# jstrom2002/Mini-OpenCL-Raytracer

Measured on AMD Instinct MI355X. Metric: Mrays/s (3840x2160 Cornell box, 8 spp, 9 bounces), higher is better.
Workload: dtype f32

## Files before the change

include/rt_hip.h:

```cpp
#ifndef RT_HIP_H
#define RT_HIP_H

#include <stddef.h>
#include <stdint.h>

#include "rt_cl_types.h"
#include "rt_status.h"

#ifdef __cplusplus
extern "C" {
#endif

typedef struct rt_context_s* rt_context;
typedef struct rt_mem_s* rt_mem;
typedef struct rt_kernel_s* rt_kernel;

#define RT_MEM_READ_WRITE (1u << 0)
#define RT_MEM_WRITE_ONLY (1u << 1)
#define RT_MEM_READ_ONLY (1u << 2)
#define RT_MEM_COPY_HOST_PTR (1u << 5)

enum rt_kernel_arg {
    RT_ARG_BUFFER_OUT = 0,
    RT_ARG_BUFFER_SCENE = 1,
// ... 329 lines not shown
typedef struct rt_rect {
    uint64_t img_offset, img_pitch, width, rows, stage_offset;
} rt_rect;
int rtBandPackPlan(unsigned width, unsigned height, unsigned period, unsigned phase, rt_rect* rects,
                   int capacity, int* n_rects, size_t* staging_bytes);

#define RT_PINNED_OP_RCP 0
#define RT_PINNED_OP_DIV 1
#define RT_PINNED_OP_SQRT 2
#define RT_PINNED_OP_RSQRT 3
#define RT_PINNED_OP_POW 4
#define RT_PINNED_OP_SIN 5
#define RT_PINNED_OP_COS 6
int rtDiagPinnedMath(int device_index, int op, const float* a, const float* b, float* out, size_t n);

const char* rtGetBuildInfo(void);

#ifdef __cplusplus
}
#endif

#endif
```

mini-opencl-raytracer_amd/clrt/_native.py:

```python
from __future__ import annotations

import ctypes
import os

import numpy as np

_PKG_ROOT = os.path.dirname(os.path.dirname(os.path.abspath(__file__)))
LIB_DIR = os.path.join(_PKG_ROOT, "lib")
HIP_LIB_PATH = os.environ.get("RT_HIP_LIB") or os.path.join(LIB_DIR, "librt_hip.so")
SCENE_LIB_PATH = os.path.join(LIB_DIR, "librt_scene.so")

RT_SUCCESS = 0
_ERROR_NAMES = {
    0: "CL_SUCCESS", -1: "CL_DEVICE_NOT_FOUND", -4: "CL_MEM_OBJECT_ALLOCATION_FAILURE",
    -5: "CL_OUT_OF_RESOURCES", -6: "CL_OUT_OF_HOST_MEMORY", -30: "CL_INVALID_VALUE",
    -33: "CL_INVALID_DEVICE", -34: "CL_INVALID_CONTEXT", -36: "CL_INVALID_COMMAND_QUEUE",
    -37: "CL_INVALID_HOST_PTR", -38: "CL_INVALID_MEM_OBJECT", -46: "CL_INVALID_KERNEL_NAME",
    -48: "CL_INVALID_KERNEL", -49: "CL_INVALID_ARG_INDEX", -50: "CL_INVALID_ARG_VALUE",
    -51: "CL_INVALID_ARG_SIZE", -52: "CL_INVALID_KERNEL_ARGS", -59: "CL_INVALID_OPERATION",
    -61: "CL_INVALID_BUFFER_SIZE", -63: "CL_INVALID_GLOBAL_WORK_SIZE",
    -1001: "RT_FILE_NOT_FOUND", -1002: "RT_PARSE_ERROR",
}


# ... 250 lines not shown
    "rtCommGetRank": (ctypes.c_int, [_vp, ctypes.POINTER(ctypes.c_int), ctypes.POINTER(ctypes.c_int)]),
    "rtCommShardKernel": (ctypes.c_int, [_vp, _vp]),
    "rtCommSetTransport": (ctypes.c_int, [_vp, ctypes.c_int]),
    "rtCommGetTransport": (ctypes.c_int, [_vp, ctypes.POINTER(ctypes.c_int), ctypes.POINTER(ctypes.c_int)]),
    "rtCommGetStatus": (ctypes.c_int, [_vp, ctypes.POINTER(CommStatus)]),
    "rtCommSetOption": (ctypes.c_int, [_vp, ctypes.c_int, ctypes.c_int]),
    "rtCommEnqueueGatherBands": (ctypes.c_int, [ctypes.POINTER(_vp), ctypes.POINTER(_vp), ctypes.c_int, ctypes.c_uint,
                                                ctypes.c_uint, ctypes.c_int, _vp]),
    "rtCommAllReduceF64": (ctypes.c_int, [ctypes.POINTER(_vp), ctypes.c_int, ctypes.POINTER(ctypes.c_double),
                                          ctypes.c_int, ctypes.c_int]),
    "rtCommBarrier": (ctypes.c_int, [ctypes.POINTER(_vp), ctypes.c_int]),
    "rtBandPackPlan": (ctypes.c_int, [ctypes.c_uint, ctypes.c_uint, ctypes.c_uint, ctypes.c_uint, ctypes.POINTER(Rect),
                                      ctypes.c_int, ctypes.POINTER(ctypes.c_int), ctypes.POINTER(ctypes.c_size_t)]),
    "rtGetBuildInfo": (ctypes.c_char_p, []),
    "rtDiagPinnedMath": (ctypes.c_int, [ctypes.c_int, ctypes.c_int, _vp, _vp, _vp, ctypes.c_size_t]),
}
HIP_EXPORTS = tuple(_HIP_PROTOS)

_SCENE_PROTOS = {
    "rtsLoadOBJ": (ctypes.c_int, [ctypes.c_char_p, ctypes.c_uint, ctypes.POINTER(_vp)]),
    "rtsLoadOBJUnbuilt": (ctypes.c_int, [ctypes.c_char_p, ctypes.POINTER(_vp)]),
    "rtsBuildFromTriangles": (ctypes.c_int, [_vp, ctypes.c_size_t, _vp, ctypes.c_size_t, ctypes.c_uint,
                                             ctypes.POINTER(_vp)]),
    "rtsGetTriangles": (ctypes.c_int, [_vp, ctypes.POINTER(_vp), ctypes.POINTER(ctypes.c_size_t)]),
    "rtsGetNodes": (ctypes.c_int, [_vp, ctypes.POINTER(_vp), ctypes.POINTER(ctypes.c_size_t)]),
    "rtsGetMaterials": (ctypes.c_int, [_vp, ctypes.POINTER(_vp), ctypes.POINTER(ctypes.c_size_t)]),
    "rtsGetTreeStats": (ctypes.c_int, [_vp, ctypes.POINTER(ctypes.c_uint), ctypes.POINTER(ctypes.c_uint),
                                       ctypes.POINTER(ctypes.c_uint)]),
    "rtsFromArrays": (ctypes.c_int, [_vp, ctypes.c_size_t, _vp, ctypes.c_size_t, _vp, ctypes.c_size_t,
                                     ctypes.c_uint, ctypes.POINTER(_vp)]),
# ... 36 lines not shown
    return _load(SCENE_LIB_PATH, _SCENE_PROTOS)


PINNED_OPS = {"rcp": 0, "div": 1, "sqrt": 2, "rsqrt": 3, "pow": 4, "sin": 5, "cos": 6}


def pinned_math(op: str, a, b=None, device: int = 0) -> np.ndarray:
    a = np.ascontiguousarray(a, dtype=np.float32)
    bb = None if b is None else np.ascontiguousarray(np.broadcast_to(np.float32(b) if np.isscalar(b) else b, a.shape),
                                                     dtype=np.float32)
    out = np.empty_like(a)
    check(hip_lib().rtDiagPinnedMath(int(device), PINNED_OPS[op], a.ctypes.data,
                                     None if bb is None else bb.ctypes.data, out.ctypes.data, a.size),
          f"pinned math {op}")
    return out
```

mini-opencl-raytracer_amd/csrc/rt_capi.cpp:

```cpp
#include <hip/hip_runtime.h>

#include <algorithm>
#include <limits>
#include <cstdlib>
#include <cstring>
#include <mutex>
#include <new>
#include <vector>

#include "../../include/rt_cl_types.h"
#include "../../include/rt_hip.h"
#include "rt_adaptive.hpp"
#include "rt_adaptive_plan.hpp"
#include "rt_bvh.hpp"
#include "rt_denoise.hpp"
#include "rt_denoise_plan.hpp"
#include "rt_denoise_samples.hpp"
#include "rt_device_scene.hpp"
#include "rt_internal.hpp"
#include "rt_kernel_state.hpp"
#include "rt_kernels.hpp"
#include "rt_launch_plan.hpp"
#include "rt_motion_launch.hpp"
#include "rt_motion_plan.hpp"
// ... 1739 lines not shown
    int count = 0;
    if (hipGetDeviceCount(&count) != hipSuccess || count == 0) return RT_DEVICE_NOT_FOUND;
    if (device_index < 0 || device_index >= count) return RT_INVALID_DEVICE;
    hipError_t e = hipSetDevice(device_index);
    float* d = nullptr;
    const size_t bytes = n * sizeof(float);
    if (e == hipSuccess) e = hipMalloc(reinterpret_cast<void**>(&d), 3 * bytes);
    if (e == hipSuccess) e = hipMemcpy(d, a, bytes, hipMemcpyHostToDevice);
    if (e == hipSuccess && two) e = hipMemcpy(d + n, b, bytes, hipMemcpyHostToDevice);
    if (e == hipSuccess) e = rtk::launch_pinned_math(op, d, d + n, d + 2 * n, n, nullptr);
    if (e == hipSuccess) e = hipMemcpy(out, d + 2 * n, bytes, hipMemcpyDeviceToHost);
    if (d) (void)hipFree(d);
    return map_hip(e);
}

const char* rtGetBuildInfo(void) {
    return "librt_hip: KernelEntry for gfx950 (HIP), math modes pinned|devicelib|shipped, scene in LDS or HBM";
}

}
```

mini-opencl-raytracer_amd/csrc/rt_kernels.hip:

```cpp
#include "rt_kernel_pick.hpp"

#pragma clang fp contract(off)

namespace rtk {

template <bool kStats, bool kBofs, int kMode>
__global__ __launch_bounds__(256) __attribute__((amdgpu_waves_per_eu(RT_STEP_DEVICELIB_WAVES, 8)))
void kernel_entry_step_devicelib_lds(KernelArgs a) {
    step_body<MathDeviceLib, true, kStats, kBofs, false, kMode>(a);
}
template <bool kStats, int kMode>
__global__ __launch_bounds__(256) __attribute__((amdgpu_waves_per_eu(RT_STEP_GLOBAL_WAVES, 8)))
void kernel_entry_step_devicelib_global(KernelArgs a) {
    step_body<MathDeviceLib, false, kStats, false, false, kMode>(a);
}
template <bool kStats, int kMode>
__global__ __launch_bounds__(256) __attribute__((amdgpu_waves_per_eu(RT_STEP_GOCT_WAVES, 8)))
void kernel_entry_step_devicelib_goct(KernelArgs a) {
    step_body<MathDeviceLib, true, kStats, false, true, kMode>(a);
}
#ifndef RT_STEP_PINNED_WAVES
#define RT_STEP_PINNED_WAVES 5
#endif
template <bool kLdsScene, bool kStats, bool kBofs, bool kGlobalOct, int kMode>
// ... 53 lines not shown
            case Walk::LdsB: return kernel_entry_step_pinned<true, S, true, false, kMode>;
            case Walk::GlobalOct: return kernel_entry_step_pinned<true, S, false, true, kMode>;
            default: return kernel_entry_step_pinned<false, S, false, false, kMode>;
        }
    }
};

template <class M>
__global__ __launch_bounds__(256) RT_ACCUM_OCC void accum_frames(KernelArgs a, const uint32_t* key) {
    accum_frames_body<M>(a, key);
}
template <class M>
__global__ void accum_key(KernelArgs a, uint32_t* key) {
    accum_key_body<M>(a, key);
}

static const Policy& policy(int math) {
    static const Policy devicelib = {pick_entry<MathDeviceLib>,   wf_pick<MathDeviceLib>,  query_pick<MathDeviceLib>,
                                     accum_frames<MathDeviceLib>, accum_key<MathDeviceLib>, camera_rays<MathDeviceLib>,
                                     pack_mats,
                                     hit_surfaces<MathDeviceLib, false>, hit_surfaces<MathDeviceLib, true>,
                                     trace_pick<MathDeviceLib>, camera_paths<MathDeviceLib>,
                                     camera_paths_for<MathDeviceLib>, sample_pick<MathDeviceLib>,
                                     motion_pick<MathDeviceLib>};
    static const Policy pinned = {pick_entry<MathPinned>,   wf_pick<MathPinned>,  query_pick<MathPinned>,
                                  accum_frames<MathPinned>, accum_key<MathPinned>, camera_rays<MathPinned>,
                                  pack_mats,
                                  hit_surfaces<MathPinned, false>, hit_surfaces<MathPinned, true>,
                                     trace_pick<MathPinned>, camera_paths<MathPinned>,
                                     camera_paths_for<MathPinned>, sample_pick<MathPinned>,
                                     motion_pick<MathPinned>};
    return math == MathShipped::kId ? shipped_policy() : math == MathDeviceLib::kId ? devicelib : pinned;
}

hipError_t launch_kernel_entry(const KernelArgs& a, const Variant& v, unsigned grid, size_t smem, hipStream_t st) {
    hipLaunchKernelGGL(policy(v.math).entry(v), dim3(grid), dim3(256), smem, st, a);
    return hipGetLastError();
}

hipError_t launch_accum_frames(const KernelArgs& a, int math, uint32_t* key, hipStream_t st) {
    const Policy& p = policy(math);
    const dim3 grid((a.nTiles + kAccumWgWaves - 1u) / kAccumWgWaves);
    hipLaunchKernelGGL(p.accum_key, dim3(1), dim3(64), 0, st, a, key);
    hipLaunchKernelGGL(p.accum_frames, grid, dim3(64 * kAccumWgWaves), 0, st, a, key);
    return hipGetLastError();
}
// ... 91 lines not shown
    if (i >= n) return;
    const float x = a[i];
    float r;
    switch (op) {
        case 0: r = MathPinned::rcp(x); break;
        case 1: r = MathPinned::div(x, b[i]); break;
        case 2: r = MathPinned::sqrt(x); break;
        case 3: r = MathPinned::rsqrt(x); break;
        case 4: r = MathPinned::pow(x, b[i]); break;
        case 5: r = MathPinned::sin(x); break;
        default: r = MathPinned::cos(x); break;
    }
    out[i] = r;
}

hipError_t launch_pinned_math(int op, const float* a, const float* b, float* out, size_t n, hipStream_t st) {
    if (n) hipLaunchKernelGGL(pinned_math_kernel, dim3((unsigned)((n + 255) / 256)), dim3(256), 0, st, op, a, b, out, n);
    return hipGetLastError();
}

hipError_t launch_pack(const rt_cl_triangle* tris, uint32_t n_tris, float4* pt, float4* ps,
                       const rt_cl_material* mats, uint32_t n_mats, float4* pm, hipStream_t st) {
    if (n_tris) hipLaunchKernelGGL(pack_tris, dim3((n_tris + 255) / 256), dim3(256), 0, st, tris, pt, n_tris);
    if (n_tris) hipLaunchKernelGGL(pack_shade, dim3((n_tris + 255) / 256), dim3(256), 0, st, tris, ps, n_tris);
    if (n_mats) hipLaunchKernelGGL(pack_mats, dim3((n_mats + 255) / 256), dim3(256), 0, st, mats, pm, n_mats);
    if (n_mats)
        hipLaunchKernelGGL(shipped_policy().pack_mats, dim3((n_mats + 255) / 256), dim3(256), 0, st, mats,
                           pm + 4 * (size_t)n_mats, n_mats);
    return hipGetLastError();
}
// ... 4 lines not shown
```

mini-opencl-raytracer_amd/csrc/rt_kernels.hpp:

```cpp
#pragma once

#include <hip/hip_runtime.h>
#include <stdint.h>

#include "../../include/rt_cl_types.h"
#include "rt_layout.hpp"
#include "rt_temporal_math.hpp"

namespace rtk {

struct KernelArgs {
    float4* result;
    const rt_cl_triangle* trisFull;
    const rt_cl_material* materials;
    const float4* packedTris;
    const float4* octNodes;
    const float4* gNodes;
    const float4* shadeTris;
    const float4* shadeMats;
    uint32_t nNodes, nTris, nMats;
    uint32_t octStride;
    uint32_t octB;
    uint32_t octRecords;
    uint32_t nTop;
// ... 110 lines not shown
struct SurfaceArgs {
    const float4* rays;
    const float4* hits;
    float4* out;
    uint32_t first, count;
    uint32_t accFirst;
    uint32_t accLast;
    float inv;
};
using SurfaceKernelFn = void (*)(KernelArgs, SurfaceArgs);
hipError_t launch_surfaces(const KernelArgs& a, const SurfaceArgs& s, int math, bool accumulate, unsigned grid,
                           hipStream_t st);

hipError_t launch_kernel_entry(const KernelArgs& a, const Variant& v, unsigned grid, size_t smem, hipStream_t st);
hipError_t launch_accum_frames(const KernelArgs& a, int math, uint32_t* key, hipStream_t st);
hipError_t launch_pinned_math(int op, const float* a, const float* b, float* out, size_t n, hipStream_t st);
hipError_t launch_pack(const rt_cl_triangle* tris, uint32_t n_tris, float4* pt, float4* ps,
                       const rt_cl_material* mats, uint32_t n_mats, float4* pm, hipStream_t st);

enum class Family : int { Entry, WfExtend, WfShade, Query, Trace, Sample, Motion };
struct OccupancyCache {
    struct Entry {
        int blocks;
        size_t smem;
    };
    Entry e[(int)Family::Motion + 1][kVariantSlots] = {};
    int get(Family f, const Variant& v, size_t smem);
};

struct Policy {
    KernelFn (*entry)(const Variant&);
    WfKernels (*wavefront)(const Variant&);
    QueryKernelFn (*query)(const Variant&);
    void (*accum_frames)(KernelArgs, const uint32_t*);
    void (*accum_key)(KernelArgs, uint32_t*);
    void (*camera_rays)(KernelArgs, float4*, uint32_t);
    void (*pack_mats)(const rt_cl_material*, float4*, uint32_t);
    SurfaceKernelFn surfaces, surfaces_accum;
    TraceKernelFn (*trace)(const Variant&);
    void (*camera_paths)(KernelArgs, float4*, uint32_t*, uint32_t);
    void (*camera_paths_for)(KernelArgs, const uint32_t*, uint32_t, uint32_t, float4*, uint32_t*);
    SampleKernelFn (*sample)(const Variant&);
    MotionKernelFn (*motion)(const Variant&);
};
const Policy& shipped_policy();
#ifndef RT_SPECIALIZE_FUSED
#define RT_SPECIALIZE_FUSED 1
#endif

}
```

mini-opencl-raytracer_amd/csrc/rt_kernels_body.hpp:

```cpp
#pragma once

#include <hip/hip_runtime.h>
#include <stdint.h>

#include "../../include/rt_cl_types.h"
#include "rt_kernels.hpp"
#include "rt_math.hpp"

#pragma clang fp contract(off)

#ifndef RT_STEP_DEVICELIB_WAVES
#define RT_STEP_DEVICELIB_WAVES 5
#endif
#ifndef RT_STEP_GLOBAL_WAVES
#define RT_STEP_GLOBAL_WAVES 6
#endif
#ifndef RT_STEP_GOCT_WAVES
#define RT_STEP_GOCT_WAVES 5
#endif

namespace rtk {

constexpr float kTwoPi = 6.28318530718f;
constexpr float kInvPi = 0.31830988618f;
// ... 518 lines not shown
    }
    return F3{M::max(radiance.x, 0.0f), M::max(radiance.y, 0.0f), M::max(radiance.z, 0.0f)};
}

template <class M>
__device__ __forceinline__ F3 gamma_out(uint32_t frameCount, F3 old, F3 rad) {
    if (frameCount == 0)
        return F3{M::pow(rad.x, 0.45454545f), M::pow(rad.y, 0.45454545f), M::pow(rad.z, 0.45454545f)};
    const float fm1 = (float)(frameCount - 1), fc = (float)frameCount;
    const F3 lin{M::pow(old.x, 2.2f), M::pow(old.y, 2.2f), M::pow(old.z, 2.2f)};
    const F3 num = madd<M>(lin, fm1, rad);
    const F3 acc{M::div(num.x, fc), M::div(num.y, fc), M::div(num.z, fc)};
    return F3{M::pow(acc.x, 0.454545f), M::pow(acc.y, 0.454545f), M::pow(acc.z, 0.454545f)};
}

template <class M>
__device__ __forceinline__ void finish_color(const KernelArgs& a, uint32_t gid, F3 rad) {
    F3 old = f3s(0.0f);
    if (a.frameCount != 0) {
        const float4 o = a.result[gid];
        old = F3{o.x, o.y, o.z};
    }
    const F3 out = gamma_out<M>(a.frameCount, old, rad);
    a.result[gid] = make_float4(out.x, out.y, out.z, 0.0f);
}

template <class M>
__device__ __forceinline__ void finish_pixel(const KernelArgs& a, uint32_t gid, F3 rad, int32_t pid,
                                             float pt) {
    finish_color<M>(a, gid, rad);
    if (a.hitIds) {
        a.hitIds[gid] = pid;
        a.hitT[gid] = pt;
    }
}

__device__ __forceinline__ unsigned long long wave_sum(uint32_t v) {
    unsigned long long x = v;
// ... 133 lines not shown

constexpr uint32_t kIdle = 0, kTrav = 1, kLeaf = 2, kShade = 3, kDone = 4;
constexpr uint32_t kNotWalking = 0x80000000u;

__device__ __forceinline__ uint32_t lane_rank(unsigned long long m) {
    return __builtin_amdgcn_mbcnt_hi((uint32_t)(m >> 32), __builtin_amdgcn_mbcnt_lo((uint32_t)m, 0u));
}

constexpr uint32_t kFinishSlots = 64;
static_assert(kFinishWaveBytes == kFinishSlots * 16, "finish queue layout");

template <class M>
__device__ __forceinline__ void finish_queued(const KernelArgs& a, const float4* fq, uint32_t n, uint32_t lane) {
    if (lane < n) {
        const float4 e = fq[lane];
        finish_color<M>(a, __float_as_uint(e.w), F3{e.x, e.y, e.z});
    }
}
#ifndef RT_PRIO_SHADE
#define RT_PRIO_SHADE 1
#endif
#ifndef RT_NODE_BURST
#define RT_NODE_BURST 7
#endif
#ifndef RT_TIMELINE
#define RT_TIMELINE 0
#endif
#ifndef RT_TIMELINE_DIV
#define RT_TIMELINE_DIV 1
#endif
#ifndef RT_TRI_BURST
#define RT_TRI_BURST 4
#endif
#ifndef RT_WTRI_BURST
#define RT_WTRI_BURST 2
#endif


// ... 131 lines not shown
    auto rootW = [&](uint32_t sgn) -> uint32_t { return kWalk ? __umul24(sgn, octStride16) : 0u; };
    if (kGlobalOct) __syncthreads();

    const F3 camPos{a.camPos[0], a.camPos[1], a.camPos[2]};
    const F3 camFront{a.camFront[0], a.camFront[1], a.camFront[2]};
    const F3 camUp{a.camUp[0], a.camUp[1], a.camUp[2]};
    const float angle = M::tan(0.5f * (45.0f * 3.1415f / 180.0f));
    const uint32_t bounces = (uint32_t)a.lightBounces;
    const uint32_t nVis = fused && kViewCull ? a.visTiles : a.nTiles;
    const uint32_t total = nVis * 64u * (fused ? a.nFrames : 1u);
    const float krad = M::max(madd<M>(1.0f, 0.5f * a.skyboxIntensity, 0.0f), 0.0f);
    float k_old = 0.0f, k_out = 0.0f;
    if (!fused && a.pfKeyIn) {
        k_old = __uint_as_float(*a.pfKeyIn);
        k_out = __uint_as_float(__builtin_amdgcn_readfirstlane(
            __float_as_uint(gamma_out<M>(a.frameCount, f3s(k_old), f3s(krad)).x)));
        if (blockIdx.x == 0 && tid == 0) *a.pfKeyOut = __float_as_uint(k_out);
    }
    const uint32_t rowEnd = a.rowBegin + a.rowCount;
    const int lane = tid & 63;
    const uint32_t kRefillMin = a.refillMin;
    const uint32_t kShadeMin = a.shadeMin;

    extern __shared__ __attribute__((aligned(16))) float4 smem[];
    float4* fq = smem + lds_scene_f4<kLdsScene, kGlobalOct>(a) + (uint32_t)(tid >> 6) * kFinishSlots;
    uint32_t fq_n = 0;
    constexpr bool kRing = kLdsScene && !kGlobalOct;
    float4* ring_d = smem + lds_scene_f4<kLdsScene, kGlobalOct>(a) + (fused ? 0u : 4u * kFinishSlots) +
                     (uint32_t)(tid >> 6) * (fused ? kRingWaveBytes / 16u : kRingWaveBytesPf / 16u);
    float4* ring_i = ring_d + kRingSlots;
    uint32_t* ring_g = reinterpret_cast<uint32_t*>(ring_d + (fused ? 2u : 1u) * kRingSlots);
// ... 291 lines not shown
            if (n_trav + n_leaf == 0u) break;
            if (n_end >= kShadeMin) break;
            const bool leaf_step = n_leaf * a.stepWeightNode > n_trav * a.stepWeightLeaf;
            if (kStats) {
                u_shadew += n_end;
                u_freew += popc_ballot(state == kIdle || state == kDone);
                u_other += leaf_step ? n_trav : n_leaf;
                if (leaf_step) {
                    ++u_tsteps;
                    u_tlanes += n_leaf;
                } else {
                    ++u_nsteps;
                    u_nlanes += n_trav;
                }
            }
            constexpr int kNodeBurst = kGlobalOct ? RT_ONODE_BURST : kLdsScene ? RT_NODE_BURST : RT_GNODE_BURST;
            constexpr int kTriBurst = kGlobalOct ? RT_OTRI_BURST : kLdsScene ? RT_TRI_BURST : RT_GTRI_BURST;
            if (!leaf_step) {
#pragma unroll
                for (int rep = 0; rep < kNodeBurst; ++rep) {
                    if (kLdsScene) {
#if RT_LDS_CONFLICTS
                        if (kStats && !kGlobalOct) {
                            const bool act = cur < kLeafMin;
                            const uint32_t i = kWalk ? cur >> 4 : __umul24(ray.sgn, a.octStride) + cur;
                            lds_model(act, i, i & 15u, true, lm[0], lm[1]);
                            const uint32_t strides[2] = {43u, 48u};
                            for (int v = 0; v < 2; ++v) {
                                const uint32_t iv = ray.sgn * strides[v] + (kWalk ? (cur >> 4) - ray.sgn * a.octStride : cur);
                                lds_model(act, iv, iv & 15u, true, lm[2 + 2 * v], lm[3 + 2 * v]);
                            }
// ... 179 lines not shown
    for (uint32_t s = 0; s < kMaxFusedFrames; ++s)
        if (s < a.nFrames) fl |= (uint32_t)a.frameFlags[(size_t)s * a.radStride + gid] << s;
    return fl;
}
__device__ __forceinline__ uint32_t load_tile_flags(const KernelArgs& a, uint32_t tile, uint32_t lane) {
    const unsigned long long* w = reinterpret_cast<const unsigned long long*>(a.frameFlags) + tile;
    uint32_t fl = 0;
#pragma unroll 1
    for (uint32_t s = 0; s < a.nFrames; ++s) fl |= (uint32_t)((w[(size_t)s * a.nTiles] >> lane) & 1ull) << s;
    return fl;
}
template <class M>
__device__ __forceinline__ F3 gamma_out_serial(uint32_t frameCount, F3 old, F3 rad) {
    if (frameCount == 0) {
        F3 o;
        o.x = M::pow(rad.x, 0.45454545f);
        __builtin_amdgcn_sched_barrier(0);
        o.y = M::pow(rad.y, 0.45454545f);
        __builtin_amdgcn_sched_barrier(0);
        o.z = M::pow(rad.z, 0.45454545f);
        return o;
    }
    const float fm1 = (float)(frameCount - 1), fc = (float)frameCount;
    float c[3] = {old.x, old.y, old.z};
    const float r[3] = {rad.x, rad.y, rad.z};
#pragma unroll
    for (int i = 0; i < 3; ++i) {
        const float lin = M::pow(c[i], 2.2f);
        __builtin_amdgcn_sched_barrier(0);
        c[i] = M::pow(M::div(madd<M>(lin, fm1, r[i]), fc), 0.454545f);
        __builtin_amdgcn_sched_barrier(0);
    }
    return F3{c[0], c[1], c[2]};
}

template <class M>
__device__ __forceinline__ F3 accum_chain_lean(const KernelArgs& a, F3 v, uint32_t gid, uint32_t flags, float krad) {
#pragma unroll 1
    for (uint32_t s = 0; s < a.nFrames; ++s) {
        const float4 r = ((flags >> s) & 1u) ? make_float4(krad, krad, krad, 0.0f)
                                             : rad_load(a.radBuf + (size_t)s * a.radStride + gid);
        v = gamma_out_serial<M>(a.frameCount + s, v, F3{r.x, r.y, r.z});
    }
    return v;
}
// ... 5 lines not shown
        const float4 r = rad_load(a.radBuf + (size_t)s * a.radStride + gid);
        if (__float_as_uint(r.x) != k || __float_as_uint(r.y) != k || __float_as_uint(r.z) != k) return 0u;
    }
    return (1u << a.nFrames) - 1u;
}

template <class M>
__device__ __forceinline__ void accum_key_body(const KernelArgs& a, uint32_t* key) {
    if (threadIdx.x != 0) return;
    if (a.workCounter) {
        a.workCounter[0] = 0u;
        a.workCounter[1] = 0u;
    }
    const float krad = M::max(madd<M>(1.0f, 0.5f * a.skyboxIntensity, 0.0f), 0.0f);
    const float kold = key[0] == 1u ? __uint_as_float(key[3]) : 0.0f;
    F3 v = f3s(kold);
    for (uint32_t s = 0; s < a.nFrames; ++s) v = gamma_out<M>(a.frameCount + s, v, f3s(krad));
    key[1] = __float_as_uint(krad);
    key[2] = __float_as_uint(kold);
    key[3] = __float_as_uint(v.x);
    key[0] = 1u;
}

#define RT_ACCUM_OCC __attribute__((amdgpu_num_vgpr(32)))
constexpr uint32_t kAccumWgWaves = 4;

template <class M>
__device__ __forceinline__ void accum_frames_body(const KernelArgs& a, const uint32_t* key) {
    const uint32_t lane = threadIdx.x & 63u, wv = threadIdx.x >> 6;
    const uint32_t kold = key[2], kout = key[3];
    const float krf = __uint_as_float(key[1]);
    const uint32_t tile = blockIdx.x * kAccumWgWaves + wv;
    if (tile >= a.nTiles) return;
    const uint32_t ty = tile / a.tilesX, tx = tile - ty * a.tilesX;
    const uint32_t x = tx * 8u + (lane & 7u), row = a.rowBegin + (ty * a.bandPeriod + a.bandPhase) * 8u + (lane >> 3);
    const uint64_t g64 = (uint64_t)row * a.width + x;
// ... 40 lines not shown
```

mini-opencl-raytracer_amd/csrc/rt_kernels_shipped.hip:

```cpp
#include "rt_kernel_pick.hpp"

#pragma clang fp contract(off)

namespace rtk {

template <bool kStats, bool kBofs, int kMode>
__global__ __launch_bounds__(256) __attribute__((amdgpu_waves_per_eu(RT_STEP_DEVICELIB_WAVES, 8)))
void kernel_entry_step_shipped_lds(KernelArgs a) {
    step_body<MathShipped, true, kStats, kBofs, false, kMode>(a);
}
template <bool kStats, int kMode>
__global__ __launch_bounds__(256) __attribute__((amdgpu_waves_per_eu(RT_STEP_GLOBAL_WAVES, 8)))
void kernel_entry_step_shipped_global(KernelArgs a) {
    step_body<MathShipped, false, kStats, false, false, kMode>(a);
}
template <bool kStats, int kMode>
__global__ __launch_bounds__(256) __attribute__((amdgpu_waves_per_eu(RT_STEP_GOCT_WAVES, 8)))
void kernel_entry_step_shipped_goct(KernelArgs a) {
    step_body<MathShipped, true, kStats, false, true, kMode>(a);
}

__global__ void pack_mats_shipped(const rt_cl_material* __restrict__ in, float4* __restrict__ out, uint32_t n) {
    const uint32_t i = blockIdx.x * blockDim.x + threadIdx.x;
    if (i >= n) return;
    material_record<MathShipped>(in[i], out + 4 * i);
}

__global__ __launch_bounds__(256) RT_ACCUM_OCC void accum_frames_shipped(KernelArgs a, const uint32_t* key) {
    accum_frames_body<MathShipped>(a, key);
}
__global__ void accum_key_shipped(KernelArgs a, uint32_t* key) {
    accum_key_body<MathShipped>(a, key);
}

template <>
struct StepEntry<MathShipped> {
    template <bool S, int kMode>
    static KernelFn get(Walk w) {
        switch (w) {
            case Walk::Lds: return kernel_entry_step_shipped_lds<S, false, kMode>;
            case Walk::LdsB: return kernel_entry_step_shipped_lds<S, true, kMode>;
            case Walk::GlobalOct: return kernel_entry_step_shipped_goct<S, kMode>;
            default: return kernel_entry_step_shipped_global<S, kMode>;
        }
    }
};

const Policy& shipped_policy() {
    static const Policy shipped = {pick_entry<MathShipped>, wf_pick<MathShipped>, query_pick<MathShipped>,
                                   accum_frames_shipped,    accum_key_shipped,    camera_rays<MathShipped>,
                                   pack_mats_shipped,
                                   hit_surfaces<MathShipped, false>, hit_surfaces<MathShipped, true>,
                                   trace_pick<MathShipped>, camera_paths<MathShipped>,
                                   camera_paths_for<MathShipped>, sample_pick<MathShipped>,
                                   motion_pick<MathShipped>};
    return shipped;
}

}
```

mini-opencl-raytracer_amd/csrc/rt_math.hpp:

```cpp
#pragma once

#include <hip/hip_runtime.h>
#include <stdint.h>

#include "../../include/rt_pinned_math.h"

#pragma clang fp contract(off)

namespace rtk {

struct F3 {
    float x, y, z;
};

__device__ __forceinline__ F3 f3(float x, float y, float z) { return F3{x, y, z}; }
__device__ __forceinline__ F3 f3s(float s) { return F3{s, s, s}; }
__device__ __forceinline__ F3 operator+(F3 a, F3 b) { return F3{a.x + b.x, a.y + b.y, a.z + b.z}; }
__device__ __forceinline__ F3 operator-(F3 a, F3 b) { return F3{a.x - b.x, a.y - b.y, a.z - b.z}; }
__device__ __forceinline__ F3 operator*(F3 a, F3 b) { return F3{a.x * b.x, a.y * b.y, a.z * b.z}; }
__device__ __forceinline__ F3 operator*(F3 a, float s) { return F3{a.x * s, a.y * s, a.z * s}; }
__device__ __forceinline__ F3 operator/(F3 a, float s) { return F3{a.x / s, a.y / s, a.z / s}; }
__device__ __forceinline__ F3 operator-(F3 a) { return F3{-a.x, -a.y, -a.z}; }

#ifndef RT_PINNED_DIAG_DIV
#define RT_PINNED_DIAG_DIV 0
#endif
#ifndef RT_PINNED_DIAG_SQRT
#define RT_PINNED_DIAG_SQRT 0
#endif
#ifndef RT_PINNED_DIAG_POW
#define RT_PINNED_DIAG_POW 0
#endif
#ifndef RT_PINNED_DIAG_TRIG
#define RT_PINNED_DIAG_TRIG 0
#endif
struct MathPinned {
    static constexpr int kId = 0;
    static constexpr bool kContract = false;
    __device__ __forceinline__ static float rcp_fast(float x) {
        const float y = __builtin_amdgcn_rcpf(x);
        return __builtin_fmaf(__builtin_fmaf(-x, y, 1.0f), y, y);
    }
#if RT_PINNED_DIAG_DIV
    __device__ __forceinline__ static float rcp(float x) { return __builtin_amdgcn_rcpf(x); }
    __device__ __forceinline__ static float div(float a, float b) { return a * __builtin_amdgcn_rcpf(b); }
#else
    __device__ __forceinline__ static float rcp(float x) {
        const float r = rcp_fast(x);
        const bool ok = (__float_as_uint(x) & 0x7fffffffu) - 0x01000000u < 0x7d000000u;
        if (__builtin_expect(__ballot(!ok) != 0ull, 0)) return ok ? r : 1.0f / x;
// ... 22 lines not shown
        if (__builtin_expect(__ballot(!ok) != 0ull, 0)) return ok ? f : pm_rsqrt(d);
        return f;
    }
#endif
    __device__ __forceinline__ static float dot(F3 a, F3 b) {
        return (a.x * b.x + a.y * b.y) + a.z * b.z;
    }
    __device__ __forceinline__ static F3 cross(F3 a, F3 b) {
        return F3{a.y * b.z - a.z * b.y, a.z * b.x - a.x * b.z, a.x * b.y - a.y * b.x};
    }
#if RT_PINNED_DIAG_POW
    __device__ __forceinline__ static float pow(float x, float y) { return ::powf(x, y); }
#else
    __device__ __forceinline__ static float pow(float x, float y) { return pm_pow(x, y); }
#endif
    __device__ __forceinline__ static float pow2(float x) { return pm_sq(x); }
#if RT_PINNED_DIAG_TRIG
    __device__ __forceinline__ static float sin(float x) { return ::sinf(x); }
    __device__ __forceinline__ static float cos(float x) { return ::cosf(x); }
    __device__ __forceinline__ static void sincos(float x, float& s, float& c) { ::sincosf(x, &s, &c); }
#else
    __device__ __forceinline__ static float sin(float x) { return pm_sin(x); }
    __device__ __forceinline__ static float cos(float x) { return pm_cos(x); }
    __device__ __forceinline__ static void sincos(float x, float& s, float& c) { pm_sincos(x, &s, &c); }
#endif
    __device__ __forceinline__ static float tan(float x) { return pm_tan(x); }
    __device__ __forceinline__ static float max(float x, float y) { return pm_max(x, y); }
    __device__ __forceinline__ static float min(float x, float y) { return pm_min(x, y); }
};

struct MathDeviceLib {
    static constexpr int kId = 1;
    static constexpr bool kContract = false;
    __device__ __forceinline__ static float rcp(float x) { return 1.0f / x; }
    __device__ __forceinline__ static float div(float a, float b) { return a / b; }
    __device__ __forceinline__ static float sqrt(float x) { return __builtin_sqrtf(x); }
    __device__ __forceinline__ static float dot(F3 a, F3 b) {
        return __builtin_fmaf(a.z, b.z, __builtin_fmaf(a.y, b.y, a.x * b.x));
    }
    __device__ __forceinline__ static F3 cross(F3 a, F3 b) {
        return F3{__builtin_fmaf(a.y, b.z, b.y * -a.z), __builtin_fmaf(a.z, b.x, b.z * -a.x),
                  __builtin_fmaf(a.x, b.y, b.x * -a.y)};
    }
    __device__ __forceinline__ static float rsqrt(float d) { return ::rsqrtf(d); }
    __device__ __forceinline__ static float pow(float x, float y) { return ::powf(x, y); }
    __device__ __forceinline__ static float pow2(float x) { return x * x; }
    __device__ __forceinline__ static float sin(float x) { return ::sinf(x); }
    __device__ __forceinline__ static float cos(float x) { return ::cosf(x); }
    __device__ __forceinline__ static void sincos(float x, float& s, float& c) { ::sincosf(x, &s, &c); }
    __device__ __forceinline__ static float tan(float x) { return ::tanf(x); }
    __device__ __forceinline__ static float max(float x, float y) { return __builtin_fmaxf(x, y); }
    __device__ __forceinline__ static float min(float x, float y) { return __builtin_fminf(x, y); }
};

struct MathShipped : MathDeviceLib {
    static constexpr int kId = 2;
    static constexpr bool kContract = true;
    __device__ __forceinline__ static float rcp(float x) {
        return __builtin_amdgcn_ldexpf(__builtin_amdgcn_rcpf(__builtin_amdgcn_frexp_mantf(x)),
                                       -__builtin_amdgcn_frexp_expf(x));
// ... 49 lines not shown
```

mini-opencl-raytracer_amd/csrc/rt_trace.hpp:

```cpp
#pragma once

namespace rtk {

constexpr uint32_t kTraceRingF4 = kTraceRingBytes / 16u;

struct TraceEnds {
    const TraceArgs& q;
    uint32_t rc_base = 0;
    uint32_t pos = 0;
    int32_t prim0 = -1;

    __device__ __forceinline__ uint32_t n_units() const { return q.nUnits; }
    __device__ __forceinline__ uint32_t fill(uint32_t u0, uint32_t lane, float4* ring, uint32_t* ring_seed) {
        rc_base = q.first + u0;
        const uint32_t rc_n = min(64u, q.count - u0);
        const float4* src = q.rays + 2 * (size_t)rc_base;
        if (lane < 2u * rc_n) ring[lane] = src[lane];
        if (lane + 64u < 2u * rc_n) ring[lane + 64u] = src[lane + 64u];
        if (lane < rc_n) ring_seed[lane] = q.seeds ? q.seeds[(size_t)rc_base + lane] : q.seedBase + (rc_base + lane);
        return rc_n;
    }
    __device__ __forceinline__ void take(uint32_t slot, const float4&) { pos = rc_base + slot; }
    __device__ __forceinline__ void unwalked() { q.out[pos] = make_float4(0.0f, 0.0f, 0.0f, __int_as_float(-1)); }
    __device__ __forceinline__ float tmin(const float4& e0) {
        prim0 = -1;
        return e0.w;
    }
    __device__ __forceinline__ void first_hit(int32_t prim) { prim0 = prim; }
    template <class M>
    __device__ __forceinline__ void finish(F3 r) {
        if (q.encoding != 0) r = gamma_out<M>(0u, f3s(0.0f), r);
        q.out[pos] = make_float4(r.x, r.y, r.z, __int_as_float(prim0));
    }
};

template <class M, bool kStats, bool kBofs, bool kGlobalOct, class Ends>
__device__ __forceinline__ void trace_loop(const KernelArgs& a, Ends& e, uint32_t refillMin, uint32_t shadeMin) {
    extern __shared__ __attribute__((aligned(16))) float4 smem[];
    const uint32_t tid = threadIdx.x, nthr = blockDim.x;
    SceneView sc;
    uint32_t scene_f4;
    if (kGlobalOct) {
        sc = SceneView{nullptr, a.packedTris, a.octNodes, a.shadeTris, a.shadeMats};
        scene_f4 = 0;
    } else {
        float4* lo = smem;
// ... 199 lines not shown
```

Measured before the change: 49620.

## Skip gamma decode on first accumulation frame and specialize gamma pow

Adds gamma-specific pow helpers that take a fast path for positive finite inputs and handle special values explicitly. When frameCount is 1 and every lane's old value is in a range where its contribution is provably zero, the pow(old, 2.2) decode is skipped wave-wide, since it gets multiplied by zero. Also lowers the LDS-scene node burst in the step kernel and adds a diagnostic kernel that exhaustively checks the pow equivalence and the skip lemma. The skip depends on a numerical lemma (pow(x,2.2)*0 == 0 for safe x) holding exactly, and the burst change alters traversal scheduling.

```diff
diff --git a/include/rt_hip.h b/include/rt_hip.h
--- a/include/rt_hip.h
+++ b/include/rt_hip.h
@@ -367,6 +367,11 @@
 #define RT_PINNED_OP_COS 6
 int rtDiagPinnedMath(int device_index, int op, const float* a, const float* b, float* out, size_t n);
 
+#define RT_GAMMA_CHECK_POW 0
+#define RT_GAMMA_CHECK_LEMMA 1
+int rtDiagGammaPow(int device_index, int math, int check, int exponent, uint32_t first, uint64_t count,
+                   uint64_t* mismatches, uint32_t* first_bad, uint32_t* first_bits);
+
 const char* rtGetBuildInfo(void);
 
 #ifdef __cplusplus
diff --git a/mini-opencl-raytracer_amd/clrt/_native.py b/mini-opencl-raytracer_amd/clrt/_native.py
--- a/mini-opencl-raytracer_amd/clrt/_native.py
+++ b/mini-opencl-raytracer_amd/clrt/_native.py
@@ -288,6 +288,8 @@
                                       ctypes.c_int, ctypes.POINTER(ctypes.c_int), ctypes.POINTER(ctypes.c_size_t)]),
     "rtGetBuildInfo": (ctypes.c_char_p, []),
     "rtDiagPinnedMath": (ctypes.c_int, [ctypes.c_int, ctypes.c_int, _vp, _vp, _vp, ctypes.c_size_t]),
+    "rtDiagGammaPow": (ctypes.c_int, [ctypes.c_int, ctypes.c_int, ctypes.c_int, ctypes.c_int, ctypes.c_uint32,
+                                      ctypes.c_uint64, _vp, _vp, _vp]),
 }
 HIP_EXPORTS = tuple(_HIP_PROTOS)
 
@@ -354,3 +356,15 @@
                                      None if bb is None else bb.ctypes.data, out.ctypes.data, a.size),
           f"pinned math {op}")
     return out
+
+
+GAMMA_EXPONENTS = {"2.2f": 0, "0.454545f": 1, "0.45454545f": 2}
+
+
+def gamma_pow_check(math: int, kind: str, exponent: str = "2.2f", first: int = 0, count: int = 1 << 32,
+                    device: int = 0):
+    bad, first_bad, bits = ctypes.c_uint64(), ctypes.c_uint32(), ctypes.c_uint32()
+    check(hip_lib().rtDiagGammaPow(int(device), int(math), {"pow": 0, "lemma": 1}[kind], GAMMA_EXPONENTS[exponent],
+                                      int(first), int(count), ctypes.byref(bad), ctypes.byref(first_bad),
+                                      ctypes.byref(bits)), "gamma pow check")
+    return bad.value, (first_bad.value if bad.value else None), bits.value
diff --git a/mini-opencl-raytracer_amd/csrc/rt_capi.cpp b/mini-opencl-raytracer_amd/csrc/rt_capi.cpp
--- a/mini-opencl-raytracer_amd/csrc/rt_capi.cpp
+++ b/mini-opencl-raytracer_amd/csrc/rt_capi.cpp
@@ -1777,6 +1777,31 @@
     return map_hip(e);
 }
 
+int rtDiagGammaPow(int device_index, int math, int check, int exponent, uint32_t first, uint64_t count,
+                   uint64_t* mismatches, uint32_t* first_bad, uint32_t* first_bits) {
+    if (math < RT_MATH_PINNED || math > RT_MATH_SHIPPED || check < RT_GAMMA_CHECK_POW || check > RT_GAMMA_CHECK_LEMMA ||
+        exponent < 0 || exponent > 2 || !mismatches || !first_bad || !first_bits)
+        return RT_INVALID_VALUE;
+    if (count > ((uint64_t)1 << 32) - first) return RT_INVALID_VALUE;
+    int ndev = 0;
+    if (hipGetDeviceCount(&ndev) != hipSuccess || ndev == 0) return RT_DEVICE_NOT_FOUND;
+    if (device_index < 0 || device_index >= ndev) return RT_INVALID_DEVICE;
+    hipError_t e = hipSetDevice(device_index);
+    unsigned long long* d = nullptr;
+    unsigned long long h[3] = {0ull, 0xffffffffull, 0ull};
+    if (e == hipSuccess) e = hipMalloc(reinterpret_cast<void**>(&d), sizeof h);
+    if (e == hipSuccess) e = hipMemcpy(d, h, sizeof h, hipMemcpyHostToDevice);
+    if (e == hipSuccess)
+        e = rtk::launch_gamma_check(rtk::GammaCheckArgs{d, count, first, (uint32_t)check, (uint32_t)exponent}, math, nullptr);
+    if (e == hipSuccess) e = hipMemcpy(h, d, sizeof h, hipMemcpyDeviceToHost);
+    if (d) (void)hipFree(d);
+    if (e != hipSuccess) return map_hip(e);
+    *mismatches = h[0];
+    *first_bad = (uint32_t)h[1];
+    *first_bits = (uint32_t)h[2];
+    return RT_SUCCESS;
+}
+
 const char* rtGetBuildInfo(void) {
     return "librt_hip: KernelEntry for gfx950 (HIP), math modes pinned|devicelib|shipped, scene in LDS or HBM";
 }
diff --git a/mini-opencl-raytracer_amd/csrc/rt_kernels.hip b/mini-opencl-raytracer_amd/csrc/rt_kernels.hip
--- a/mini-opencl-raytracer_amd/csrc/rt_kernels.hip
+++ b/mini-opencl-raytracer_amd/csrc/rt_kernels.hip
@@ -91,6 +91,10 @@
 __global__ void accum_key(KernelArgs a, uint32_t* key) {
     accum_key_body<M>(a, key);
 }
+template <class M>
+__global__ __launch_bounds__(256) void gamma_check(GammaCheckArgs g) {
+    gamma_check_body<M>(g);
+}
 
 static const Policy& policy(int math) {
     static const Policy devicelib = {pick_entry<MathDeviceLib>,   wf_pick<MathDeviceLib>,  query_pick<MathDeviceLib>,
@@ -99,14 +103,14 @@
                                      hit_surfaces<MathDeviceLib, false>, hit_surfaces<MathDeviceLib, true>,
                                      trace_pick<MathDeviceLib>, camera_paths<MathDeviceLib>,
                                      camera_paths_for<MathDeviceLib>, sample_pick<MathDeviceLib>,
-                                     motion_pick<MathDeviceLib>};
+                                     motion_pick<MathDeviceLib>, gamma_check<MathDeviceLib>};
     static const Policy pinned = {pick_entry<MathPinned>,   wf_pick<MathPinned>,  query_pick<MathPinned>,
                                   accum_frames<MathPinned>, accum_key<MathPinned>, camera_rays<MathPinned>,
                                   pack_mats,
                                   hit_surfaces<MathPinned, false>, hit_surfaces<MathPinned, true>,
                                      trace_pick<MathPinned>, camera_paths<MathPinned>,
                                      camera_paths_for<MathPinned>, sample_pick<MathPinned>,
-                                     motion_pick<MathPinned>};
+                                     motion_pick<MathPinned>, gamma_check<MathPinned>};
     return math == MathShipped::kId ? shipped_policy() : math == MathDeviceLib::kId ? devicelib : pinned;
 }
 
@@ -228,6 +232,11 @@
     out[i] = r;
 }
 
+hipError_t launch_gamma_check(const GammaCheckArgs& g, int math, hipStream_t st) {
+    if (g.count) hipLaunchKernelGGL(policy(math).gamma_check, dim3(256u * 8u), dim3(256), 0, st, g);
+    return hipGetLastError();
+}
+
 hipError_t launch_pinned_math(int op, const float* a, const float* b, float* out, size_t n, hipStream_t st) {
     if (n) hipLaunchKernelGGL(pinned_math_kernel, dim3((unsigned)((n + 255) / 256)), dim3(256), 0, st, op, a, b, out, n);
     return hipGetLastError();
diff --git a/mini-opencl-raytracer_amd/csrc/rt_kernels.hpp b/mini-opencl-raytracer_amd/csrc/rt_kernels.hpp
--- a/mini-opencl-raytracer_amd/csrc/rt_kernels.hpp
+++ b/mini-opencl-raytracer_amd/csrc/rt_kernels.hpp
@@ -148,6 +148,14 @@
 
 hipError_t launch_kernel_entry(const KernelArgs& a, const Variant& v, unsigned grid, size_t smem, hipStream_t st);
 hipError_t launch_accum_frames(const KernelArgs& a, int math, uint32_t* key, hipStream_t st);
+struct GammaCheckArgs {
+    unsigned long long* out;
+    unsigned long long count;
+    uint32_t first;
+    uint32_t check;
+    uint32_t exponent;
+};
+hipError_t launch_gamma_check(const GammaCheckArgs& g, int math, hipStream_t st);
 hipError_t launch_pinned_math(int op, const float* a, const float* b, float* out, size_t n, hipStream_t st);
 hipError_t launch_pack(const rt_cl_triangle* tris, uint32_t n_tris, float4* pt, float4* ps,
                        const rt_cl_material* mats, uint32_t n_mats, float4* pm, hipStream_t st);
@@ -176,6 +184,7 @@
     void (*camera_paths_for)(KernelArgs, const uint32_t*, uint32_t, uint32_t, float4*, uint32_t*);
     SampleKernelFn (*sample)(const Variant&);
     MotionKernelFn (*motion)(const Variant&);
+    void (*gamma_check)(GammaCheckArgs);
 };
 const Policy& shipped_policy();
 #ifndef RT_SPECIALIZE_FUSED
diff --git a/mini-opencl-raytracer_amd/csrc/rt_kernels_body.hpp b/mini-opencl-raytracer_amd/csrc/rt_kernels_body.hpp
--- a/mini-opencl-raytracer_amd/csrc/rt_kernels_body.hpp
+++ b/mini-opencl-raytracer_amd/csrc/rt_kernels_body.hpp
@@ -556,14 +556,41 @@
     return F3{M::pow(acc.x, 0.454545f), M::pow(acc.y, 0.454545f), M::pow(acc.z, 0.454545f)};
 }
 
-template <class M>
+__device__ __forceinline__ bool gamma_old_safe(float v) {
+    const uint32_t b = __float_as_uint(v);
+    return b <= 0x5C000000u || b == 0x80000000u;
+}
+__device__ __forceinline__ bool gamma_skip_from(uint32_t frameCount, F3 old) {
+    if (!RT_GAMMA_FAST || __builtin_amdgcn_readfirstlane(frameCount) != 1u) return false;
+    return __ballot(!(gamma_old_safe(old.x) && gamma_old_safe(old.y) && gamma_old_safe(old.z))) == 0ull;
+}
+template <class M>
+__device__ __forceinline__ float gamma_out_step1(uint32_t frameCount, float old, float rad, bool skip) {
+    if (frameCount == 0) return M::template pow_gamma<GammaExp::kTo0>(rad);
+    const float fm1 = (float)(frameCount - 1), fc = (float)frameCount;
+    float lin = 0.0f;
+    if (!skip) lin = M::template pow_gamma<GammaExp::kFrom>(old);
+    return M::template pow_gamma<GammaExp::kTo>(M::div(madd<M>(lin, fm1, rad), fc));
+}
+template <class M>
+__device__ __forceinline__ F3 gamma_out_step(uint32_t frameCount, F3 old, F3 rad) {
+    const bool skip = gamma_skip_from(frameCount, old);
+    return F3{gamma_out_step1<M>(frameCount, old.x, rad.x, skip), gamma_out_step1<M>(frameCount, old.y, rad.y, skip),
+              gamma_out_step1<M>(frameCount, old.z, rad.z, skip)};
+}
+template <class M>
+__device__ __forceinline__ float gamma_out_key(uint32_t frameCount, float old, float rad) {
+    return gamma_out_step1<M>(frameCount, old, rad, gamma_skip_from(frameCount, f3s(old)));
+}
+
+template <class M, bool kStep = false>
 __device__ __forceinline__ void finish_color(const KernelArgs& a, uint32_t gid, F3 rad) {
     F3 old = f3s(0.0f);
     if (a.frameCount != 0) {
         const float4 o = a.result[gid];
         old = F3{o.x, o.y, o.z};
     }
-    const F3 out = gamma_out<M>(a.frameCount, old, rad);
+    const F3 out = kStep ? gamma_out_step<M>(a.frameCount, old, rad) : gamma_out<M>(a.frameCount, old, rad);
     a.result[gid] = make_float4(out.x, out.y, out.z, 0.0f);
 }
 
@@ -727,7 +754,7 @@
 __device__ __forceinline__ void finish_queued(const KernelArgs& a, const float4* fq, uint32_t n, uint32_t lane) {
     if (lane < n) {
         const float4 e = fq[lane];
-        finish_color<M>(a, __float_as_uint(e.w), F3{e.x, e.y, e.z});
+        finish_color<M, true>(a, __float_as_uint(e.w), F3{e.x, e.y, e.z});
     }
 }
 #ifndef RT_PRIO_SHADE
@@ -735,6 +762,9 @@
 #endif
 #ifndef RT_NODE_BURST
 #define RT_NODE_BURST 7
+#endif
+#ifndef RT_STEP_NODE_BURST
+#define RT_STEP_NODE_BURST 5
 #endif
 #ifndef RT_TIMELINE
 #define RT_TIMELINE 0
@@ -896,7 +926,7 @@
     if (!fused && a.pfKeyIn) {
         k_old = __uint_as_float(*a.pfKeyIn);
         k_out = __uint_as_float(__builtin_amdgcn_readfirstlane(
-            __float_as_uint(gamma_out<M>(a.frameCount, f3s(k_old), f3s(krad)).x)));
+            __float_as_uint(gamma_out_key<M>(a.frameCount, k_old, krad))));
         if (blockIdx.x == 0 && tid == 0) *a.pfKeyOut = __float_as_uint(k_out);
     }
     const uint32_t rowEnd = a.rowBegin + a.rowCount;
@@ -1218,7 +1248,7 @@
                     u_nlanes += n_trav;
                 }
             }
-            constexpr int kNodeBurst = kGlobalOct ? RT_ONODE_BURST : kLdsScene ? RT_NODE_BURST : RT_GNODE_BURST;
+            constexpr int kNodeBurst = kGlobalOct ? RT_ONODE_BURST : kLdsScene ? RT_STEP_NODE_BURST : RT_GNODE_BURST;
             constexpr int kTriBurst = kGlobalOct ? RT_OTRI_BURST : kLdsScene ? RT_TRI_BURST : RT_GTRI_BURST;
             if (!leaf_step) {
 #pragma unroll
@@ -1428,21 +1458,29 @@
 __device__ __forceinline__ F3 gamma_out_serial(uint32_t frameCount, F3 old, F3 rad) {
     if (frameCount == 0) {
         F3 o;
-        o.x = M::pow(rad.x, 0.45454545f);
+        o.x = M::template pow_gamma<GammaExp::kTo0>(rad.x);
         __builtin_amdgcn_sched_barrier(0);
-        o.y = M::pow(rad.y, 0.45454545f);
+        o.y = M::template pow_gamma<GammaExp::kTo0>(rad.y);
         __builtin_amdgcn_sched_barrier(0);
-        o.z = M::pow(rad.z, 0.45454545f);
+        o.z = M::template pow_gamma<GammaExp::kTo0>(rad.z);
         return o;
     }
     const float fm1 = (float)(frameCount - 1), fc = (float)frameCount;
     float c[3] = {old.x, old.y, old.z};
     const float r[3] = {rad.x, rad.y, rad.z};
+    if (gamma_skip_from(frameCount, old)) {
+#pragma unroll
+        for (int i = 0; i < 3; ++i) {
+            c[i] = M::template pow_gamma<GammaExp::kTo>(M::div(madd<M>(0.0f, fm1, r[i]), fc));
+            __builtin_amdgcn_sched_barrier(0);
+        }
+        return F3{c[0], c[1], c[2]};
+    }
 #pragma unroll
     for (int i = 0; i < 3; ++i) {
-        const float lin = M::pow(c[i], 2.2f);
+        const float lin = M::template pow_gamma<GammaExp::kFrom>(c[i]);
         __builtin_amdgcn_sched_barrier(0);
-        c[i] = M::pow(M::div(madd<M>(lin, fm1, r[i]), fc), 0.454545f);
+        c[i] = M::template pow_gamma<GammaExp::kTo>(M::div(madd<M>(lin, fm1, r[i]), fc));
         __builtin_amdgcn_sched_barrier(0);
     }
     return F3{c[0], c[1], c[2]};
@@ -1478,12 +1516,46 @@
     }
     const float krad = M::max(madd<M>(1.0f, 0.5f * a.skyboxIntensity, 0.0f), 0.0f);
     const float kold = key[0] == 1u ? __uint_as_float(key[3]) : 0.0f;
-    F3 v = f3s(kold);
-    for (uint32_t s = 0; s < a.nFrames; ++s) v = gamma_out<M>(a.frameCount + s, v, f3s(krad));
+    float v = kold;
+    for (uint32_t s = 0; s < a.nFrames; ++s) v = gamma_out_key<M>(a.frameCount + s, v, krad);
     key[1] = __float_as_uint(krad);
     key[2] = __float_as_uint(kold);
-    key[3] = __float_as_uint(v.x);
+    key[3] = __float_as_uint(v);
     key[0] = 1u;
+}
+
+template <class M, GammaExp E>
+__device__ __forceinline__ void gamma_check_one(uint32_t check, uint32_t b, uint32_t& got, uint32_t& want) {
+    const float x = __uint_as_float(b);
+    if (check == 0u) {
+        got = __float_as_uint(M::template pow_gamma<E>(x));
+        want = __float_as_uint(M::pow(x, gamma_exp<E>()));
+    } else {
+        got = __float_as_uint(M::pow(x, 2.2f) * 0.0f);
+        want = 0u;
+    }
+}
+template <class M>
+__device__ __forceinline__ void gamma_check_body(const GammaCheckArgs& g) {
+    const uint64_t stride = (uint64_t)gridDim.x * blockDim.x;
+    unsigned long long bad = 0ull;
+    uint32_t firstBad = 0xffffffffu;
+    for (uint64_t i = (uint64_t)blockIdx.x * blockDim.x + threadIdx.x; i < g.count; i += stride) {
+        const uint32_t b = g.first + (uint32_t)i;
+        uint32_t got, want;
+        if (g.exponent == 0u) gamma_check_one<M, GammaExp::kFrom>(g.check, b, got, want);
+        else if (g.exponent == 1u) gamma_check_one<M, GammaExp::kTo>(g.check, b, got, want);
+        else gamma_check_one<M, GammaExp::kTo0>(g.check, b, got, want);
+        if (i == 0u) g.out[2] = got;
+        if (got != want) {
+            ++bad;
+            firstBad = firstBad < b ? firstBad : b;
+        }
+    }
+    if (bad != 0ull) {
+        atomicAdd(reinterpret_cast<unsigned long long*>(g.out), bad);
+        atomicMin(reinterpret_cast<uint32_t*>(g.out + 1), firstBad);
+    }
 }
 
 #define RT_ACCUM_OCC __attribute__((amdgpu_num_vgpr(32)))
diff --git a/mini-opencl-raytracer_amd/csrc/rt_kernels_shipped.hip b/mini-opencl-raytracer_amd/csrc/rt_kernels_shipped.hip
--- a/mini-opencl-raytracer_amd/csrc/rt_kernels_shipped.hip
+++ b/mini-opencl-raytracer_amd/csrc/rt_kernels_shipped.hip
@@ -32,6 +32,7 @@
 __global__ void accum_key_shipped(KernelArgs a, uint32_t* key) {
     accum_key_body<MathShipped>(a, key);
 }
+__global__ __launch_bounds__(256) void gamma_check_shipped(GammaCheckArgs g) { gamma_check_body<MathShipped>(g); }
 
 template <>
 struct StepEntry<MathShipped> {
@@ -53,7 +54,7 @@
                                    hit_surfaces<MathShipped, false>, hit_surfaces<MathShipped, true>,
                                    trace_pick<MathShipped>, camera_paths<MathShipped>,
                                    camera_paths_for<MathShipped>, sample_pick<MathShipped>,
-                                   motion_pick<MathShipped>};
+                                   motion_pick<MathShipped>, gamma_check_shipped};
     return shipped;
 }
 
diff --git a/mini-opencl-raytracer_amd/csrc/rt_math.hpp b/mini-opencl-raytracer_amd/csrc/rt_math.hpp
--- a/mini-opencl-raytracer_amd/csrc/rt_math.hpp
+++ b/mini-opencl-raytracer_amd/csrc/rt_math.hpp
@@ -34,6 +34,15 @@
 #ifndef RT_PINNED_DIAG_TRIG
 #define RT_PINNED_DIAG_TRIG 0
 #endif
+#ifndef RT_GAMMA_FAST
+#define RT_GAMMA_FAST 1
+#endif
+enum class GammaExp { kFrom, kTo, kTo0 };
+template <GammaExp E>
+__device__ __forceinline__ constexpr float gamma_exp() {
+    return E == GammaExp::kFrom ? 2.2f : E == GammaExp::kTo ? 0.454545f : 0.45454545f;
+}
+
 struct MathPinned {
     static constexpr int kId = 0;
     static constexpr bool kContract = false;
@@ -86,6 +95,10 @@
 #else
     __device__ __forceinline__ static float pow(float x, float y) { return pm_pow(x, y); }
 #endif
+    template <GammaExp E>
+    __device__ __forceinline__ static float pow_gamma(float x) {
+        return pow(x, gamma_exp<E>());
+    }
     __device__ __forceinline__ static float pow2(float x) { return pm_sq(x); }
 #if RT_PINNED_DIAG_TRIG
     __device__ __forceinline__ static float sin(float x) { return ::sinf(x); }
@@ -116,6 +129,20 @@
     }
     __device__ __forceinline__ static float rsqrt(float d) { return ::rsqrtf(d); }
     __device__ __forceinline__ static float pow(float x, float y) { return ::powf(x, y); }
+    template <GammaExp E>
+    __device__ __forceinline__ static float pow_gamma(float x) {
+#if RT_GAMMA_FAST
+        if (x > 0.0f && x < __builtin_inff() && !(x == 1.0f)) return ::powf(x, gamma_exp<E>());
+        const uint32_t b = __float_as_uint(x), mag = b & 0x7fffffffu;
+        float r = __uint_as_float(0x7fc00000u);
+        if (b == 0x3f800000u) r = 1.0f;
+        if (mag == 0u) r = 0.0f;
+        if (mag == 0x7f800000u) r = __builtin_inff();
+        return r;
+#else
+        return ::powf(x, gamma_exp<E>());
+#endif
+    }
     __device__ __forceinline__ static float pow2(float x) { return x * x; }
     __device__ __forceinline__ static float sin(float x) { return ::sinf(x); }
     __device__ __forceinline__ static float cos(float x) { return ::cosf(x); }
diff --git a/mini-opencl-raytracer_amd/csrc/rt_trace.hpp b/mini-opencl-raytracer_amd/csrc/rt_trace.hpp
--- a/mini-opencl-raytracer_amd/csrc/rt_trace.hpp
+++ b/mini-opencl-raytracer_amd/csrc/rt_trace.hpp
@@ -29,7 +29,7 @@
     __device__ __forceinline__ void first_hit(int32_t prim) { prim0 = prim; }
     template <class M>
     __device__ __forceinline__ void finish(F3 r) {
-        if (q.encoding != 0) r = gamma_out<M>(0u, f3s(0.0f), r);
+        if (q.encoding != 0) r = gamma_out_step<M>(0u, f3s(0.0f), r);
         q.out[pos] = make_float4(r.x, r.y, r.z, __int_as_float(prim0));
     }
 };
```

Result: faster. 50850, median of 6 (+2.5%).
